# ToKe79/nuts333

Measured on AMD Instinct MI355X. Metric: delivered_broadcast_lines_per_s, higher is better.
Workload: dtype u8

## Files before the change

nuts333_amd/device/fanout.hip:

```cpp

#include <hip/hip_runtime.h>
#include <hipcub/hipcub.hpp>

#include <algorithm>
#include <chrono>
#include <cstdint>
#include <cstdio>
#include <cstring>
#include <type_traits>

namespace {

constexpr int kOutBuff = 1000;
constexpr int kTextSize = 2000;
constexpr int kNumCols = 21;
constexpr int kMaxWrites = 16;
constexpr int kBlock = 256;

constexpr uint8_t kLogin = 1, kHasRoom = 2, kSameRoom = 4, kIgnall = 8, kIgnshout = 16, kSender = 32, kColour = 64;
constexpr int kComShout = 4, kComSemote = 7;

__constant__ char kColCom[kNumCols][2] = {
    {'R', 'S'}, {'O', 'L'}, {'U', 'L'}, {'L', 'I'}, {'R', 'V'}, {'F', 'K'}, {'F', 'R'}, {'F', 'G'}, {'F', 'Y'}, {'F', 'B'},
    {'F', 'M'}, {'F', 'T'}, {'F', 'W'}, {'B', 'K'}, {'B', 'R'}, {'B', 'G'}, {'B', 'Y'}, {'B', 'B'}, {'B', 'M'}, {'B', 'T'},
    {'B', 'W'},
};
__constant__ char kColArg[kNumCols][2] = {
    {'0', 0}, {'1', 0}, {'4', 0}, {'5', 0}, {'7', 0}, {'3', '0'}, {'3', '1'}, {'3', '2'}, {'3', '3'}, {'3', '4'},
    {'3', '5'}, {'3', '6'}, {'3', '7'}, {'4', '0'}, {'4', '1'}, {'4', '2'}, {'4', '3'}, {'4', '4'}, {'4', '5'}, {'4', '6'},
    {'4', '7'},
};

__device__ __forceinline__ bool admits(uint8_t l, int rm_is_null, int force_listen, int com_num)
{
    if (l & kLogin) return false;
    if (!(l & kHasRoom)) return false;
    if (!(l & kSameRoom) && !rm_is_null) return false;
    if ((l & kIgnall) && !force_listen) return false;
    if ((l & kIgnshout) && (com_num == kComShout || com_num == kComSemote)) return false;
    if (l & kSender) return false;
    return true;
}

__device__ __forceinline__ int colcom_at(const uint8_t* s, int i, int len)
{
    if (i + 2 >= len) return -1;
    const uint8_t a = s[i + 1], b = s[i + 2];
    for (int c = 0; c < kNumCols; c++)
        if (a == (uint8_t)kColCom[c][0] && b == (uint8_t)kColCom[c][1]) return c;
    return -1;
}

template <bool EMIT>
struct Sink {
    uint8_t* out;
    int32_t* wsz;
    int64_t cap;
    int wcap;
    int64_t n = 0;
    int writes = 0;
    int pos = 0;

    __device__ __forceinline__ void put(uint8_t c)
    {
        if (EMIT && n < cap) out[n] = c;
        n++;
        pos++;
    }
    __device__ __forceinline__ void flush()
    {
        if (EMIT && writes < wcap) wsz[writes] = pos;
        writes++;
        pos = 0;
    }
    __device__ __forceinline__ void reset_code()
    {
        put(27); put('['); put('0'); put('m');
    }
};

template <bool EMIT>
__device__ void transduce(const uint8_t* s, int len, bool colour, Sink<EMIT>& k)
{
    int i = 0;
    while (i < len) {
        const uint8_t ch = s[i];
        if (ch == '\n') {
            if (k.pos > kOutBuff - 6) k.flush();
            if (colour) k.reset_code();
            k.put('\n');
            k.put('\r');
            i++;
        } else if (ch == '/' && i + 1 < len && s[i + 1] == '~') {
            i++;
            continue;
        } else if (i > 0 && ch == '~' && s[i - 1] == '/') {
            k.put('~');
            i++;
        } else if (ch == '~') {
            if (k.pos > kOutBuff - 6) k.flush();
            const int c = colcom_at(s, i, len);
            if (c >= 0) {
                if (colour) {
                    k.put(27); k.put('['); k.put((uint8_t)kColArg[c][0]);
                    if (kColArg[c][1]) k.put((uint8_t)kColArg[c][1]);
                    k.put('m');
                }
                i += 3;
            } else {
                k.put('~');
                i++;
            }
        } else {
            k.put(ch);
            i++;
        }
        if (k.pos == kOutBuff) k.flush();
    }
    if (k.pos) k.flush();
    if (colour) {
        k.reset_code();
        k.flush();
    }
}

struct Args {
    const uint8_t* text;
    const int32_t* text_off;
    const int32_t* text_len;
    const uint8_t* rec;
    int n;
    int rm_is_null, force_listen, com_num;
    uint8_t* admitted;
    int64_t* nbytes;
    int32_t* nwrites;
    int64_t* out_off;
    int32_t* w_off;
    int* violations;
    uint8_t* arena;
    int64_t arena_cap;
    int32_t* wsz;
    int64_t wsz_cap;
};

template <bool BROADCAST>
__device__ __forceinline__ bool load_item(const Args& a, int i, const uint8_t*& s, int& len)
{
    if (BROADCAST) {
        __shared__ uint8_t lds[kTextSize];
        len = a.text_len[0];
        for (int j = threadIdx.x; j < len; j += blockDim.x) lds[j] = a.text[j];
        __syncthreads();
        s = lds;
        return i < a.n;
    }
    if (i >= a.n) return false;
    s = a.text + a.text_off[i];
    len = a.text_len[i];
    return true;
}

template <bool BROADCAST>
__device__ void measure(const Args& a)
{
    const int i = blockIdx.x * blockDim.x + threadIdx.x;
    if (i == 0) {
        a.nbytes[a.n] = 0;
        a.nwrites[a.n] = 0;
    }
    const uint8_t* s;
    int len;
    if (!load_item<BROADCAST>(a, i, s, len)) return;
    const uint8_t l = a.rec[i];
    const bool in = !BROADCAST || admits(l, a.rm_is_null, a.force_listen, a.com_num);
    Sink<false> k{nullptr, nullptr, 0, 0};
    if (in) transduce(s, len, (l & kColour) != 0, k);
    if (k.n > 6 * (int64_t)len + 4 || k.writes > kMaxWrites) atomicAdd(a.violations, 1);
    a.admitted[i] = in;
    a.nbytes[i] = k.n;
    a.nwrites[i] = k.writes;
}

template <bool BROADCAST>
__device__ void emit(const Args& a)
{
    const int i = blockIdx.x * blockDim.x + threadIdx.x;
    const uint8_t* s;
    int len;
    if (!load_item<BROADCAST>(a, i, s, len) || !a.admitted[i]) return;
    const int64_t room = a.arena_cap - a.out_off[i], wroom = a.wsz_cap - a.w_off[i];
    const int64_t cap = a.nbytes[i] < room ? a.nbytes[i] : (room > 0 ? room : 0);
    const int wcap = (int)(a.nwrites[i] < wroom ? a.nwrites[i] : (wroom > 0 ? wroom : 0));
    Sink<true> k{a.arena + a.out_off[i], a.wsz + a.w_off[i], cap, wcap};
    transduce(s, len, (a.rec[i] & kColour) != 0, k);
}

constexpr int kVarCap = 6 * (kTextSize - 1) + 4;
constexpr int kGroup = 16;

struct ManyArgs {
    const uint8_t* text;
    const int32_t* text_off;
    const int32_t* text_len;
    const uint8_t* flags;
    const int32_t* com_num;
    const int32_t* item_off;
    const int32_t* tile_off;
    const uint8_t* rec;
    int k, m;
    int* violations;
    uint8_t* admitted;
    int64_t* out_off;
    int32_t* w_off;
    int64_t* nbytes;
    int32_t* nwrites;
    uint8_t* arena;
    int64_t arena_cap;
    int32_t* wsz;
    int64_t wsz_cap;
};

struct Tile {
    int b, lo, hi;
};

__device__ __forceinline__ Tile find_tile(const ManyArgs& a)
{
    const int blk = (int)blockIdx.x;
    int lo = 0, hi = a.k;
    while (hi - lo > 1) {
        const int mid = (lo + hi) >> 1;
        if (a.tile_off[mid] <= blk) lo = mid;
        else hi = mid;
    }
    const int first = a.item_off[lo] + (blk - a.tile_off[lo]) * kBlock;
    const int end = a.item_off[lo + 1];
    return {lo, first, first + kBlock < end ? first + kBlock : end};
}

template <bool EMIT, typename A>
__device__ __forceinline__ void stage_variants(const A& a, int b, uint8_t* text, uint8_t* var, int32_t* vwsz,
                                               int64_t* vn, int* vw)
{
    const int len = a.text_len[b];
    const uint8_t* src = a.text + a.text_off[b];
    for (int j = threadIdx.x; j < len; j += blockDim.x) text[j] = src[j];
    __syncthreads();
    if (threadIdx.x == 0 || threadIdx.x == 64) {
        const int c = threadIdx.x >> 6;
        Sink<EMIT> k{EMIT ? var + c * kVarCap : nullptr, EMIT ? vwsz + c * kMaxWrites : nullptr, 6 * (int64_t)len + 4,
                     kMaxWrites};
        transduce(text, len, c != 0, k);
        vn[c] = k.n;
        vw[c] = k.writes;
    }
    __syncthreads();
}

__device__ void measure_many(const ManyArgs& a)
{
    __shared__ uint8_t text[kTextSize];
    __shared__ int64_t vn[2];
    __shared__ int vw[2];
    if (blockIdx.x == 0 && threadIdx.x == 0) {
        a.nbytes[a.m] = 0;
        a.nwrites[a.m] = 0;
    }
    const Tile t = find_tile(a);
    stage_variants<false>(a, t.b, text, nullptr, nullptr, vn, vw);
    const int i = t.lo + (int)threadIdx.x;
    if (i >= t.hi) return;
    const uint8_t l = a.rec[i];
    const int fl = a.flags[t.b];
    const bool in = admits(l, fl & 1, (fl >> 1) & 1, a.com_num[t.b]);
    const int c = (l & kColour) ? 1 : 0;
    const int64_t nb = in ? vn[c] : 0;
    const int nw = in ? vw[c] : 0;
    if (nb > 6 * (int64_t)a.text_len[t.b] + 4 || nw > kMaxWrites) atomicAdd(a.violations, 1);
    a.admitted[i] = in;
    a.nbytes[i] = nb;
    a.nwrites[i] = nw;
}

__device__ void emit_many(const ManyArgs& a)
{
    __shared__ uint8_t text[kTextSize];
    __shared__ uint8_t var[2 * kVarCap];
    __shared__ int32_t vwsz[2 * kMaxWrites];
    __shared__ int64_t vn[2];
    __shared__ int vw[2];
    __shared__ int64_t s_off[kBlock], s_n[kBlock];
    __shared__ int32_t s_woff[kBlock], s_nw[kBlock];
    __shared__ uint8_t s_c[kBlock];
    const Tile t = find_tile(a);
    const int len = a.text_len[t.b];
    {
        const int i = t.lo + (int)threadIdx.x;
        if (i < t.hi) {
            const bool in = a.admitted[i] != 0;
            const int64_t off = a.out_off[i], woff = a.w_off[i];
            const int64_t room = a.arena_cap - off, wroom = a.wsz_cap - woff;
            int64_t n = in ? a.nbytes[i] : 0;
            n = n < room ? n : room;
            n = n < 6 * (int64_t)len + 4 ? n : 6 * (int64_t)len + 4;
            int64_t nw = in ? a.nwrites[i] : 0;
            nw = nw < wroom ? nw : wroom;
            nw = nw < kMaxWrites ? nw : kMaxWrites;
            s_off[threadIdx.x] = off;
            s_n[threadIdx.x] = n > 0 ? n : 0;
            s_woff[threadIdx.x] = (int32_t)woff;
            s_nw[threadIdx.x] = nw > 0 ? (int32_t)nw : 0;
            s_c[threadIdx.x] = (a.rec[i] & kColour) ? 1 : 0;
        }
    }
    stage_variants<true>(a, t.b, text, var, vwsz, vn, vw);
    const int g = (int)threadIdx.x / kGroup, lane = (int)threadIdx.x % kGroup;
    for (int j = g; j < t.hi - t.lo; j += kBlock / kGroup) {
        const int c = s_c[j];
        const int64_t n0 = s_n[j], vmax = vn[c] < kVarCap ? vn[c] : kVarCap;
        const int64_t n = n0 < vmax ? n0 : vmax;
        const uint8_t* src = var + c * kVarCap;
        uint8_t* dst = a.arena + s_off[j];
        const int head = (int)(s_off[j] & 3);
        for (int64_t w = 4 * lane - head; w < n; w += 4 * kGroup) {
            if (w >= 0 && w + 4 <= n) {
                const uint32_t v = (uint32_t)src[w] | (uint32_t)src[w + 1] << 8 | (uint32_t)src[w + 2] << 16 |
                                   (uint32_t)src[w + 3] << 24;
                *reinterpret_cast<uint32_t*>(dst + w) = v;
            } else {
                for (int q = 0; q < 4; q++)
                    if (w + q >= 0 && w + q < n) dst[w + q] = src[w + q];
            }
        }
        const int nw = s_nw[j] < vw[c] ? s_nw[j] : vw[c];
        if (lane < nw) a.wsz[s_woff[j] + lane] = vwsz[c * kMaxWrites + lane];
    }
}

static_assert(kGroup >= kMaxWrites, "emit_many writes an item's chunk sizes with one lane each");
static_assert(kBlock % kGroup == 0 && kBlock >= 128, "emit_many: whole lane groups; variants on waves 0 and 1");

struct RosterArgs {
    const int32_t* room;
    const uint8_t* slot;
    const uint8_t* text;
    const int32_t* text_off;
    const int32_t* text_len;
    const int32_t* rm;
    const int32_t* sender;
    const uint8_t* flags;
    const int32_t* com_num;
    int k, capacity, tiles;
    int* violations;
    uint8_t* admitted;
    int64_t* out_off;
    int32_t* w_off;
    uint8_t* var;
    int64_t* vn;
    int32_t* vw;
    int32_t* vwsz;
    uint8_t* arena;
    int64_t arena_cap;
    int32_t* wsz;
    int64_t wsz_cap;
};

__host__ __device__ __forceinline__ int64_t var_stride(int len) { return (6 * (int64_t)len + 4 + 3) & ~(int64_t)3; }
__device__ __forceinline__ int64_t var_at(const RosterArgs& a, int b) { return 12 * (int64_t)a.text_off[b] + 16 * (int64_t)b; }

__device__ void roster_measure(const RosterArgs& a)
{
    const int b = (int)blockIdx.x / a.tiles, tile = (int)blockIdx.x - b * a.tiles;
    const int j = tile * kBlock + (int)threadIdx.x;
    if (j < a.capacity) {
        const int room = a.room[j], rm = a.rm[b];
        const uint8_t l = (a.slot[j] & (kLogin | kIgnall | kIgnshout | kColour)) | (room >= 0 ? kHasRoom : 0) |
                          (rm >= 0 && room == rm ? kSameRoom : 0) | (j == a.sender[b] ? kSender : 0);
        a.admitted[b * a.capacity + j] = admits(l, rm < 0, (a.flags[b] >> 1) & 1, a.com_num[b]);
    }
    if (tile == 0) {
        __shared__ uint8_t text[kTextSize];
        __shared__ uint8_t var[2 * kVarCap];
        __shared__ int32_t vwsz[2 * kMaxWrites];
        __shared__ int64_t vn[2];
        __shared__ int vw[2];
        stage_variants<true>(a, b, text, var, vwsz, vn, vw);
        const int len = a.text_len[b];
        const int64_t cap = 6 * (int64_t)len + 4, stride = var_stride(len);
        uint8_t* dst = a.var + var_at(a, b);
        for (int c = 0; c < 2; c++) {
            const int64_t n = vn[c] < cap ? vn[c] : cap;
            for (int64_t q = threadIdx.x; q < n; q += kBlock) dst[c * stride + q] = var[c * kVarCap + q];
            const int nw = vw[c] < kMaxWrites ? vw[c] : kMaxWrites;
            if ((int)threadIdx.x < nw) a.vwsz[(2 * b + c) * kMaxWrites + threadIdx.x] = vwsz[c * kMaxWrites + threadIdx.x];
        }
        if (threadIdx.x < 2) {
            a.vn[2 * b + threadIdx.x] = vn[threadIdx.x];
            a.vw[2 * b + threadIdx.x] = vw[threadIdx.x];
            if (vn[threadIdx.x] > cap || vw[threadIdx.x] > kMaxWrites) atomicAdd(a.violations, 1);
        }
    }
}

template <typename T>
struct ItemCount {
    const uint8_t* admitted;
    const uint8_t* slot;
    const T* v;
    int capacity, m;
    __host__ __device__ T operator()(int i) const
    {
        if (i >= m || !admitted[i]) return 0;
        const int b = i / capacity;
        return v[2 * b + ((slot[i - b * capacity] & kColour) ? 1 : 0)];
    }
};

__device__ __forceinline__ void copy_items(int count, const uint8_t* var, const int32_t* vwsz, const int64_t* vn,
                                           const int* vw, const int64_t* s_off, const int64_t* s_n,
                                           const int32_t* s_woff, const int32_t* s_nw, const uint8_t* s_c,
                                           uint8_t* arena, int32_t* wsz)
{
    const int g = (int)threadIdx.x / kGroup, lane = (int)threadIdx.x % kGroup;
    for (int j = g; j < count; j += kBlock / kGroup) {
        const int c = s_c[j];
        const int64_t n0 = s_n[j], vmax = vn[c] < kVarCap ? vn[c] : kVarCap;
        const int64_t n = n0 < vmax ? n0 : vmax;
        const uint8_t* src = var + c * kVarCap;
        uint8_t* dst = arena + s_off[j];
        const int head = (int)(s_off[j] & 3);
        for (int64_t w = 4 * lane - head; w < n; w += 4 * kGroup) {
            if (w >= 0 && w + 4 <= n) {
                const uint32_t v = (uint32_t)src[w] | (uint32_t)src[w + 1] << 8 | (uint32_t)src[w + 2] << 16 |
                                   (uint32_t)src[w + 3] << 24;
                *reinterpret_cast<uint32_t*>(dst + w) = v;
            } else {
                for (int q = 0; q < 4; q++)
                    if (w + q >= 0 && w + q < n) dst[w + q] = src[w + q];
            }
        }
        const int nw = s_nw[j] < vw[c] ? s_nw[j] : vw[c];
        if (lane < nw) wsz[s_woff[j] + lane] = vwsz[c * kMaxWrites + lane];
    }
}

__device__ void roster_emit(const RosterArgs& a)
{
    __shared__ uint8_t var[2 * kVarCap];
    __shared__ int32_t vwsz[2 * kMaxWrites];
    __shared__ int64_t vn[2];
    __shared__ int vw[2];
    __shared__ int64_t s_off[kBlock], s_n[kBlock];
    __shared__ int32_t s_woff[kBlock], s_nw[kBlock];
    __shared__ uint8_t s_c[kBlock];
    const int b = (int)blockIdx.x / a.tiles, j0 = ((int)blockIdx.x - b * a.tiles) * kBlock;
    const int len = a.text_len[b];
    const int64_t cap = 6 * (int64_t)len + 4;
    {
        const int j = j0 + (int)threadIdx.x;
        if (j < a.capacity) {
            const int i = b * a.capacity + j;
            const bool in = a.admitted[i] != 0;
            const int64_t off = a.out_off[i], woff = a.w_off[i];
            const int64_t room = a.arena_cap - off, wroom = a.wsz_cap - woff;
            int64_t n = in ? a.out_off[i + 1] - off : 0;
            n = n < room ? n : room;
            n = n < cap ? n : cap;
            int64_t nw = in ? a.w_off[i + 1] - woff : 0;
            nw = nw < wroom ? nw : wroom;
            nw = nw < kMaxWrites ? nw : kMaxWrites;
            s_off[threadIdx.x] = off;
            s_n[threadIdx.x] = n > 0 ? n : 0;
            s_woff[threadIdx.x] = (int32_t)woff;
            s_nw[threadIdx.x] = nw > 0 ? (int32_t)nw : 0;
            s_c[threadIdx.x] = (a.slot[j] & kColour) ? 1 : 0;
        }
    }
    const uint8_t* src = a.var + var_at(a, b);
    const int64_t stride = var_stride(len);
    for (int c = 0; c < 2; c++) {
        const int64_t n = a.vn[2 * b + c] < cap ? a.vn[2 * b + c] : cap;
        for (int64_t q = threadIdx.x; q < n; q += kBlock) var[c * kVarCap + q] = src[c * stride + q];
        const int nw = a.vw[2 * b + c] < kMaxWrites ? a.vw[2 * b + c] : kMaxWrites;
        if ((int)threadIdx.x < nw) vwsz[c * kMaxWrites + threadIdx.x] = a.vwsz[(2 * b + c) * kMaxWrites + threadIdx.x];
        if (threadIdx.x == 0) {
            vn[c] = n;
            vw[c] = nw;
        }
    }
    __syncthreads();
    const int count = a.capacity - j0 < kBlock ? a.capacity - j0 : kBlock;
    copy_items(count, var, vwsz, vn, vw, s_off, s_n, s_woff, s_nw, s_c, a.arena, a.wsz);
}

static_assert(2 * kMaxWrites <= kBlock, "roster kernels move a broadcast's chunk sizes with one lane each");

struct PlanArgs {
    const int32_t* room;
    const uint8_t* slot;
    const uint8_t* text;
    const int32_t* text_off;
    const int32_t* text_len;
    const int32_t* rm;
    const int32_t* sender;
    const uint8_t* flags;
    const int32_t* com_num;
    int k, capacity, tiles;
    int words;
    int* violations;
    int64_t* vn;
    int32_t* vw;
    int32_t* vwsz;
    uint64_t* bits;
    uint8_t* var;
};

__device__ __forceinline__ int64_t var_at(const PlanArgs& a, int b) { return 12 * (int64_t)a.text_off[b] + 16 * (int64_t)b; }

__device__ void roster_plan(const PlanArgs& a)
{
    const int b = (int)blockIdx.x / a.tiles, tile = (int)blockIdx.x - b * a.tiles;
    const int j = tile * kBlock + (int)threadIdx.x;
    bool in = false;
    if (j < a.capacity) {
        const int room = a.room[j], rm = a.rm[b];
        const uint8_t l = (a.slot[j] & (kLogin | kIgnall | kIgnshout | kColour)) | (room >= 0 ? kHasRoom : 0) |
                          (rm >= 0 && room == rm ? kSameRoom : 0) | (j == a.sender[b] ? kSender : 0);
        in = admits(l, rm < 0, (a.flags[b] >> 1) & 1, a.com_num[b]);
    }
    const uint64_t word = __ballot(in);
    const int w = j >> 6;
    if ((threadIdx.x & 63) == 0 && w < a.words) a.bits[(int64_t)b * a.words + w] = word;
    if (tile == 0) {
        __shared__ uint8_t text[kTextSize];
        __shared__ uint8_t var[2 * kVarCap];
        __shared__ int32_t vwsz[2 * kMaxWrites];
        __shared__ int64_t vn[2];
        __shared__ int vw[2];
        stage_variants<true>(a, b, text, var, vwsz, vn, vw);
        const int len = a.text_len[b];
        const int64_t cap = 6 * (int64_t)len + 4, stride = var_stride(len);
        uint8_t* dst = a.var + var_at(a, b);
        for (int c = 0; c < 2; c++) {
            const int64_t n = vn[c] < cap ? vn[c] : cap;
            for (int64_t q = threadIdx.x; q < n; q += kBlock) dst[c * stride + q] = var[c * kVarCap + q];
            const int nw = vw[c] < kMaxWrites ? vw[c] : kMaxWrites;
            if ((int)threadIdx.x < nw) a.vwsz[(2 * b + c) * kMaxWrites + threadIdx.x] = vwsz[c * kMaxWrites + threadIdx.x];
        }
        if (threadIdx.x < 2) {
            a.vn[2 * b + threadIdx.x] = vn[threadIdx.x];
            a.vw[2 * b + threadIdx.x] = vw[threadIdx.x];
            if (vn[threadIdx.x] > cap || vw[threadIdx.x] > kMaxWrites) atomicAdd(a.violations, 1);
        }
    }
}

static_assert(kBlock % 64 == 0, "roster_plan: a tile is whole bitmap words, one per wave");

constexpr int kRevLines = 15;
constexpr int kRevLen = 200;
constexpr int kRevSlot = kRevLen + 2;
constexpr int kRevRing = kRevLines * kRevSlot;
constexpr int kRevLineCap = 6 * (kRevLen + 1) + 4;
constexpr int kRevLineStride = (kRevLineCap + 1 + 3) & ~3;
constexpr int kRevLineWrites = 3;
constexpr int kRevVarCap = kRevLines * kRevLineCap;
constexpr int kRevVarStride = (kRevVarCap + 3) & ~3;
constexpr int kRevWrites = kRevLines * kRevLineWrites;
constexpr int kRevTasks = 2 * kRevLines;
constexpr int kWaveLimit = kOutBuff - 6;
constexpr uint8_t kRecordBit = 4;
constexpr int kMaxReviewRooms = 1024;

struct RecordArgs {
    const uint8_t* text;
    const int32_t* text_off;
    const int32_t* text_len;
    const int32_t* rm;
    const uint8_t* flags;
    const uint8_t* clear;
    int k, review_rooms;
    uint8_t* rings;
    int32_t* revline;
};

__device__ void roster_record(const RecordArgs& a)
{
    __shared__ int s_surv[kRevLines];
    __shared__ int s_count, s_base;
    const int room = (int)blockIdx.x;
    const bool cleared = a.clear && a.clear[room];
    if (threadIdx.x < 64) {
        const int lane = (int)threadIdx.x;
        int count = 0;
        for (int b0 = 0; b0 < a.k; b0 += 64) {
            const int b = b0 + lane;
            const bool hit = b < a.k && (a.flags[b] & kRecordBit) && a.rm[b] == room;
            const uint64_t word = __ballot(hit);
            const int n = __popcll(word);
            const int rank = count + __popcll(word & ((1ull << lane) - 1));
            if (hit && rank >= count + n - kRevLines) s_surv[rank % kRevLines] = b;
            count += n;
        }
        if (lane == 0) {
            s_count = count;
            s_base = cleared ? 0 : (int)((uint32_t)a.revline[room] % kRevLines);
        }
    }
    __syncthreads();
    const int count = s_count, base = s_base;
    if (!count && !cleared) return;
    uint8_t* ring = a.rings + (size_t)room * kRevRing;
    const int nsurv = count < kRevLines ? count : kRevLines;
    const int first = (count - nsurv) % kRevLines;
    if (cleared && threadIdx.x < kRevLines) {
        const int d = ((int)threadIdx.x - base - first + 2 * kRevLines) % kRevLines;
        if (d >= nsurv) ring[threadIdx.x * kRevSlot] = 0;
    }
    for (int idx = (int)threadIdx.x; idx < nsurv * kRevSlot; idx += kBlock) {
        const int j = idx / kRevSlot, i = idx - j * kRevSlot;
        const int r = (first + j) % kRevLines;
        const int b = s_surv[r];
        uint8_t v = 0;
        if (i < kRevLen) {
            if (i < a.text_len[b]) v = a.text[a.text_off[b] + i];
        } else if (i == kRevLen) {
            v = '\n';
        }
        ring[((base + r) % kRevLines) * kRevSlot + i] = v;
    }
    if (threadIdx.x == 0) a.revline[room] = (base + count % kRevLines) % kRevLines;
}

struct ReviewArgs {
    uint8_t* rings;
    int32_t* revline;
    const int32_t* rooms;
    const uint8_t* clear;
    int q, review_rooms;
    int* violations;
    int32_t* line_count;
    int32_t* sequential;
    int32_t* vn;
    int32_t* vw;
    int32_t* vwsz;
    uint8_t* lines;
    uint8_t* var;
};

__device__ __forceinline__ int expand_byte(uint8_t p1, uint8_t ch, uint8_t n1, bool consumed, int own, bool colour,
                                           uint64_t* v)
{
    *v = ch;
    if (ch == 0 || consumed) return 0;
    if (ch == '\n') {
        if (colour) {
            *v = 27ull | (uint64_t)'[' << 8 | (uint64_t)'0' << 16 | (uint64_t)'m' << 24 | (uint64_t)'\n' << 32 |
                 (uint64_t)'\r' << 40;
            return 6;
        }
        *v = (uint64_t)'\n' | (uint64_t)'\r' << 8;
        return 2;
    }
    if (ch == '/' && n1 == '~') return 0;
    if (ch == '~' && p1 != '/' && own >= 0) {
        if (!colour) return 0;
        const uint64_t a0 = (uint8_t)kColArg[own][0], a1 = (uint8_t)kColArg[own][1];
        *v = 27ull | (uint64_t)'[' << 8 | a0 << 16 | (a1 ? a1 << 24 | (uint64_t)'m' << 32 : (uint64_t)'m' << 24);
        return a1 ? 5 : 4;
    }
    return 1;
}

__device__ void roster_review(const ReviewArgs& a)
{
    if ((int)blockIdx.x >= a.q) {
        const int room = ((int)blockIdx.x - a.q) * kBlock + (int)threadIdx.x;
        if (a.clear && room < a.review_rooms && a.clear[room]) {
            for (int i = 0; i < kRevLines; i++) a.rings[(size_t)room * kRevRing + i * kRevSlot] = 0;
            a.revline[room] = 0;
        }
        return;
    }
    __shared__ uint8_t s_line[kRevLines][kRevSlot + 2];
    __shared__ uint8_t s_out[kRevTasks][kRevLineStride];
    __shared__ int32_t s_wsz[kRevTasks][kRevLineWrites + 1];
    __shared__ int s_n[kRevTasks], s_w[kRevTasks], s_off[kRevTasks], s_woff[kRevTasks];
    __shared__ int s_len[kRevLines], s_seq;
    const int q = (int)blockIdx.x, room = a.rooms[q];
    const bool cleared = a.clear && a.clear[room];
    const int rev = cleared ? 0 : (int)((uint32_t)a.revline[room] % kRevLines);
    const uint8_t* ring = a.rings + (size_t)room * kRevRing;
    for (int idx = (int)threadIdx.x; idx < kRevRing; idx += kBlock) {
        const int i = idx / kRevSlot, j = idx - i * kRevSlot;
        const uint8_t v = cleared ? 0 : ring[((rev + i) % kRevLines) * kRevSlot + j];
        s_line[i][j] = v;
        a.lines[(size_t)q * kRevRing + idx] = v;
    }
    if (threadIdx.x == 0) s_seq = 0;
    __syncthreads();

    const int lane = (int)threadIdx.x & 63;
    for (int t = (int)threadIdx.x >> 6; t < kRevTasks; t += kBlock / 64) {
        const int i = t >> 1;
        const bool colour = (t & 1) != 0;
        const uint8_t* s = s_line[i];
        uint8_t w[9];
#pragma unroll
        for (int x = 0; x < 9; x++) {
            const int at = 4 * lane - 3 + x;
            w[x] = at >= 0 && at < kRevSlot ? s[at] : 0;
        }
        const int nul = w[3] == 0 ? 0 : w[4] == 0 ? 1 : w[5] == 0 ? 2 : w[6] == 0 ? 3 : 4;
        const uint64_t ends = __ballot(nul < 4);
        const int end_lane = __ffsll((unsigned long long)ends) - 1;
        const int len = 4 * end_lane + __shfl(nul, end_lane, 64);
#pragma unroll
        for (int x = 0; x < 9; x++)
            if (4 * lane - 3 + x >= len) w[x] = 0;
        int cmd[6], key[6];
        bool tilde = false;
#pragma unroll
        for (int x = 0; x < 6; x++) {
            cmd[x] = -1;
            key[x] = w[x + 1] == '~' && w[x] != '/' ? w[x + 2] << 8 | w[x + 3] : -1;
            tilde |= key[x] >= 0;
        }
        if (tilde) {
#pragma unroll 1
            for (int c = 0; c < kNumCols; c++) {
                const int pair = (uint8_t)kColCom[c][0] << 8 | (uint8_t)kColCom[c][1];
#pragma unroll
                for (int x = 0; x < 6; x++) cmd[x] = key[x] == pair ? c : cmd[x];
            }
        }
        int n[4], mine = 0;
        uint64_t v[4];
#pragma unroll
        for (int x = 0; x < 4; x++) {
            n[x] = expand_byte(w[x + 2], w[x + 3], w[x + 4], cmd[x] >= 0 || cmd[x + 1] >= 0, cmd[x + 2], colour, &v[x]);
            mine += n[x];
        }
        int incl = mine;
#pragma unroll
        for (int d = 1; d < 64; d <<= 1) {
            const int y = __shfl_up(incl, d, 64);
            if (lane >= d) incl += y;
        }
        const int body = __shfl(incl, 63, 64);
        uint8_t* out = s_out[t];
        if (len == 0) {
            if (lane == 0) {
                s_n[t] = 0;
                s_w[t] = 0;
            }
        } else if (body <= kWaveLimit) {
            int at = incl - mine;
#pragma unroll
            for (int x = 0; x < 4; x++) {
#pragma unroll
                for (int y = 0; y < 6; y++)
                    out[y < n[x] ? at + y : kRevLineStride - 1] = (uint8_t)(v[x] >> (8 * y));
                at += n[x];
            }
            if (colour && lane < 4) out[body + lane] = lane == 0 ? 27 : lane == 1 ? '[' : lane == 2 ? '0' : 'm';
            if (lane == 0) {
                int nw = 0;
                if (body) s_wsz[t][nw++] = body;
                if (colour) s_wsz[t][nw++] = 4;
                s_n[t] = body + (colour ? 4 : 0);
                s_w[t] = nw;
            }
        } else if (lane == 0) {
            s_n[t] = -1;
        }
        if (lane == 0 && !colour) s_len[i] = len;
    }
    __syncthreads();
    if (threadIdx.x < kRevTasks && s_n[threadIdx.x] < 0) {
        const int t = (int)threadIdx.x;
        Sink<true> k{s_out[t], s_wsz[t], kRevLineCap, kRevLineWrites};
        transduce(s_line[t >> 1], s_len[t >> 1], (t & 1) != 0, k);
        if (k.n > kRevLineCap || k.writes > kRevLineWrites) atomicAdd(a.violations, 1);
        s_n[t] = k.n < kRevLineCap ? (int)k.n : kRevLineCap;
        s_w[t] = k.writes < kRevLineWrites ? k.writes : kRevLineWrites;
        atomicAdd(&s_seq, 1);
    }
    __syncthreads();
    if (threadIdx.x < kRevTasks) {
        const int t = (int)threadIdx.x;
        int off = 0, woff = 0;
        for (int j = t & 1; j < t; j += 2) {
            off += s_n[j];
            woff += s_w[j];
        }
        s_off[t] = off;
        s_woff[t] = woff;
        if (t >= kRevTasks - 2) {
            a.vn[2 * q + (t & 1)] = off + s_n[t];
            a.vw[2 * q + (t & 1)] = woff + s_w[t];
        }
    }
    if (threadIdx.x == 64) {
        int lines = 0;
        for (int i = 0; i < kRevLines; i++) lines += s_len[i] > 0;
        a.line_count[q] = lines;
        a.sequential[q] = s_seq;
    }
    __syncthreads();
    for (int t = 0; t < kRevTasks; t++) {
        const int var = 2 * q + (t & 1);
        uint8_t* dst = a.var + (size_t)var * kRevVarStride + s_off[t];
        for (int j = (int)threadIdx.x; j < s_n[t]; j += kBlock) dst[j] = s_out[t][j];
        if ((int)threadIdx.x < s_w[t]) a.vwsz[var * kRevWrites + s_woff[t] + (int)threadIdx.x] = s_wsz[t][threadIdx.x];
    }
}

static_assert(kBlock / 64 >= 1 && 64 * 4 >= kRevSlot, "roster_review: a wave holds a whole slot, four bytes per lane");
static_assert(kBlock >= kRevTasks + 64 && kBlock >= kRevLines, "roster_review / roster_record: a lane per task, per line");

}

extern "C" __global__ void __launch_bounds__(kBlock) nuts_fanout_measure_batch(Args a) { measure<false>(a); }
extern "C" __global__ void __launch_bounds__(kBlock) nuts_fanout_measure_broadcast(Args a) { measure<true>(a); }
extern "C" __global__ void __launch_bounds__(kBlock) nuts_fanout_emit_batch(Args a) { emit<false>(a); }
extern "C" __global__ void __launch_bounds__(kBlock) nuts_fanout_emit_broadcast(Args a) { emit<true>(a); }
extern "C" __global__ void __launch_bounds__(kBlock) nuts_fanout_measure_many(ManyArgs a) { measure_many(a); }
extern "C" __global__ void __launch_bounds__(kBlock) nuts_fanout_emit_many(ManyArgs a) { emit_many(a); }
extern "C" __global__ void __launch_bounds__(kBlock) nuts_roster_measure(RosterArgs a) { roster_measure(a); }
extern "C" __global__ void __launch_bounds__(kBlock) nuts_roster_emit(RosterArgs a) { roster_emit(a); }
extern "C" __global__ void __launch_bounds__(kBlock) nuts_roster_plan(PlanArgs a) { roster_plan(a); }
extern "C" __global__ void __launch_bounds__(kBlock) nuts_roster_record(RecordArgs a) { roster_record(a); }
extern "C" __global__ void __launch_bounds__(kBlock) nuts_roster_review(ReviewArgs a) { roster_review(a); }


namespace {

struct Buffers {
    uint8_t* d_block = nullptr;
    size_t cap_block = 0, cap_host_arena = 0, cap_host_writes = 0;
    uint8_t* h_arena = nullptr;
    int32_t* h_wsz = nullptr;
    hipStream_t stream = nullptr;
    hipEvent_t ev0 = nullptr, ev1 = nullptr;
    bool ready = false;
};
Buffers g;
char g_err[512];

int fail(const char* what, hipError_t e)
{
    snprintf(g_err, sizeof(g_err), "%s: %s", what, hipGetErrorString(e));
    return -1;
}

#define ND_CHECK(call)                                  \
    do {                                                \
        hipError_t e_ = (call);                         \
        if (e_ != hipSuccess) return fail(#call, e_);   \
    } while (0)

template <typename T>
int grow_dev(T** p, size_t* cap, size_t want, const char* what)
{
    if (want <= *cap) return 0;
    if (*p) (void)hipFree(*p);
    *p = nullptr;
    *cap = 0;
    hipError_t e = hipMalloc((void**)p, want * sizeof(T));
    if (e != hipSuccess) return fail(what, e);
    *cap = want;
    return 0;
}

template <typename T>
int grow_host(T** p, size_t* cap, size_t want, const char* what)
{
    if (want <= *cap) return 0;
    if (*p) (void)hipHostFree(*p);
    *p = nullptr;
    *cap = 0;
    hipError_t e = hipHostMalloc((void**)p, want * sizeof(T), hipHostMallocDefault);
    if (e != hipSuccess) return fail(what, e);
    *cap = want;
    return 0;
}

int ensure_ready()
{
    if (g.ready) return 0;
    int n = 0;
    ND_CHECK(hipGetDeviceCount(&n));
    if (n < 1) {
        snprintf(g_err, sizeof(g_err), "no GPU visible");
        return -1;
    }
    ND_CHECK(hipSetDevice(0));
    ND_CHECK(hipStreamCreateWithFlags(&g.stream, hipStreamNonBlocking));
    ND_CHECK(hipEventCreate(&g.ev0));
    ND_CHECK(hipEventCreate(&g.ev1));
    g.ready = true;
    return 0;
}

size_t layout(uintptr_t base, size_t text_bytes, size_t scan_bytes, Args& a, uint8_t** scan)
{
    size_t at = 0;
    auto take = [&](auto*& p, size_t count) {
        p = reinterpret_cast<std::remove_reference_t<decltype(p)>>(base + at);
        at += (count * sizeof(*p) + 255) & ~(size_t)255;
    };
    const size_t n = (size_t)a.n;
    take(a.text, text_bytes);
    take(a.text_off, n);
    take(a.text_len, n);
    take(a.rec, n);
    take(a.admitted, n);
    take(a.nbytes, n + 1);
    take(a.nwrites, n + 1);
    take(a.out_off, n + 1);
    take(a.w_off, n + 1);
    take(a.violations, 1);
    take(a.arena, (size_t)a.arena_cap);
    take(a.wsz, (size_t)a.wsz_cap);
    take(*scan, scan_bytes);
    return at;
}

double now_ns()
{
    return (double)std::chrono::duration_cast<std::chrono::nanoseconds>(
               std::chrono::steady_clock::now().time_since_epoch()).count();
}

struct ManyHost {
    uint8_t* stage = nullptr;
    uint8_t* res = nullptr;
    size_t cap_stage = 0, cap_res = 0;
};
ManyHost gm;

size_t layout_many(uintptr_t base, size_t text_bytes, size_t scan_bytes, ManyArgs& a, uint8_t** scan)
{
    size_t at = 0;
    auto take = [&](auto*& p, size_t count) {
        p = reinterpret_cast<std::remove_reference_t<decltype(p)>>(base + at);
        at += (count * sizeof(*p) + 255) & ~(size_t)255;
    };
    const size_t k = (size_t)a.k, m = (size_t)a.m;
    take(a.text, text_bytes);
    take(a.text_off, k);
    take(a.text_len, k);
    take(a.flags, k);
    take(a.com_num, k);
    take(a.item_off, k + 1);
    take(a.tile_off, k + 1);
    take(a.rec, m);
    take(a.violations, 1);
    take(a.admitted, m);
    take(a.out_off, m + 1);
    take(a.w_off, m + 1);
    take(a.nbytes, m + 1);
    take(a.nwrites, m + 1);
    take(a.arena, (size_t)a.arena_cap);
    take(a.wsz, (size_t)a.wsz_cap);
    take(*scan, scan_bytes);
    return at;
}

constexpr int kMaxRosters = 64;
constexpr int kMaxCapacity = 65536;
struct Roster {
    bool live = false;
    bool resident = false;
    int capacity = 0;
    int64_t rooms = 0;
    uint8_t* d = nullptr;
    uint8_t* mirror = nullptr;
    size_t cap_d = 0, cap_mirror = 0;
    int review_rooms = 0;
    uint8_t* rings = nullptr;
};
Roster g_rosters[kMaxRosters];

size_t revline_at(const Roster& r) { return ((size_t)r.review_rooms * kRevRing + 255) & ~(size_t)255; }
size_t rings_bytes(const Roster& r) { return revline_at(r) + (size_t)r.review_rooms * sizeof(int32_t); }

size_t layout_roster(uintptr_t base, size_t text_bytes, RosterArgs& a)
{
    size_t at = 0;
    auto take = [&](auto*& p, size_t count) {
        p = reinterpret_cast<std::remove_reference_t<decltype(p)>>(base + at);
        at += (count * sizeof(*p) + 255) & ~(size_t)255;
    };
    const size_t k = (size_t)a.k, m = k * (size_t)a.capacity;
    take(a.room, (size_t)a.capacity);
    take(a.slot, (size_t)a.capacity);
    take(a.text, text_bytes);
    take(a.text_off, k);
    take(a.text_len, k);
    take(a.rm, k);
    take(a.sender, k);
    take(a.flags, k);
    take(a.com_num, k);
    take(a.violations, 1);
    take(a.admitted, m);
    take(a.out_off, m + 1);
    take(a.w_off, m + 1);
    return at;
}

size_t layout_roster_work(uintptr_t base, size_t var_bytes, size_t scan_bytes, RosterArgs& a, uint8_t** scan)
{
    size_t at = 0;
    auto take = [&](auto*& p, size_t count) {
        p = reinterpret_cast<std::remove_reference_t<decltype(p)>>(base + at);
        at += (count * sizeof(*p) + 255) & ~(size_t)255;
    };
    const size_t k = (size_t)a.k;
    take(a.var, var_bytes);
    take(a.vn, 2 * k);
    take(a.vw, 2 * k);
    take(a.vwsz, 2 * k * kMaxWrites);
    take(a.arena, (size_t)a.arena_cap);
    take(a.wsz, (size_t)a.wsz_cap);
    take(*scan, scan_bytes);
    return at;
}

size_t layout_plan(uintptr_t base, size_t text_bytes, size_t var_bytes, PlanArgs& a, size_t clear_bytes,
                   const uint8_t** clear)
{
    size_t at = 0;
    auto take = [&](auto*& p, size_t count) {
        p = reinterpret_cast<std::remove_reference_t<decltype(p)>>(base + at);
        at += (count * sizeof(*p) + 255) & ~(size_t)255;
    };
    const size_t k = (size_t)a.k;
    take(a.room, (size_t)a.capacity);
    take(a.slot, (size_t)a.capacity);
    take(a.text, text_bytes);
    take(a.text_off, k);
    take(a.text_len, k);
    take(a.rm, k);
    take(a.sender, k);
    take(a.flags, k);
    take(a.com_num, k);
    take(*clear, clear_bytes);
    take(a.violations, 1);
    take(a.vn, 2 * k);
    take(a.vw, 2 * k);
    take(a.vwsz, 2 * k * kMaxWrites);
    take(a.bits, k * (size_t)a.words);
    take(a.var, var_bytes);
    return at;
}

size_t layout_review(uintptr_t base, int capacity, size_t clear_bytes, ReviewArgs& a)
{
    size_t at = 0;
    auto take = [&](auto*& p, size_t count) {
        p = reinterpret_cast<std::remove_reference_t<decltype(p)>>(base + at);
        at += (count * sizeof(*p) + 255) & ~(size_t)255;
    };
    const size_t q = (size_t)a.q;
    const int32_t* room;
    const uint8_t* slot;
// ... 605 lines not shown
```

Measured before the change: 733,300.

## Parallelize broadcast text transduction across a wave with prefix-sum scatter

Replaces the single-thread serial transducer used to stage each broadcast's plain and colour variants with a 64-lane wave version. Each lane expands 4 bytes, looks up colour codes branch-free, and computes output offsets via a shuffle prefix sum, with the serial path kept as fallback when output exceeds one write buffer. The review path is refactored to share the same helper, and the fallback uses a branch-free colour-code lookup. This removes a long serial per-block stage at the cost of more lanes busy and extra shuffle work; outputs must match the serial write-splitting semantics.

```diff
diff --git a/nuts333_amd/device/fanout.hip b/nuts333_amd/device/fanout.hip
--- a/nuts333_amd/device/fanout.hip
+++ b/nuts333_amd/device/fanout.hip
@@ -12,6 +12,7 @@
 namespace {
 
 constexpr int kOutBuff = 1000;
+constexpr int kWaveLimit = kOutBuff - 6;
 constexpr int kTextSize = 2000;
 constexpr int kNumCols = 21;
 constexpr int kMaxWrites = 16;
@@ -42,13 +43,21 @@
     return true;
 }
 
+template <bool LADDER = true>
 __device__ __forceinline__ int colcom_at(const uint8_t* s, int i, int len)
 {
     if (i + 2 >= len) return -1;
     const uint8_t a = s[i + 1], b = s[i + 2];
+    if (LADDER) {
+        for (int c = 0; c < kNumCols; c++)
+            if (a == (uint8_t)kColCom[c][0] && b == (uint8_t)kColCom[c][1]) return c;
+        return -1;
+    }
+    int found = -1;
+#pragma unroll
     for (int c = 0; c < kNumCols; c++)
-        if (a == (uint8_t)kColCom[c][0] && b == (uint8_t)kColCom[c][1]) return c;
-    return -1;
+        found = (a << 8 | b) == ((uint8_t)kColCom[c][0] << 8 | (uint8_t)kColCom[c][1]) ? c : found;
+    return found;
 }
 
 template <bool EMIT>
@@ -79,7 +88,7 @@
     }
 };
 
-template <bool EMIT>
+template <bool EMIT, bool LADDER = true>
 __device__ void transduce(const uint8_t* s, int len, bool colour, Sink<EMIT>& k)
 {
     int i = 0;
@@ -99,7 +108,7 @@
             i++;
         } else if (ch == '~') {
             if (k.pos > kOutBuff - 6) k.flush();
-            const int c = colcom_at(s, i, len);
+            const int c = colcom_at<LADDER>(s, i, len);
             if (c >= 0) {
                 if (colour) {
                     k.put(27); k.put('['); k.put((uint8_t)kColArg[c][0]);
@@ -122,6 +131,87 @@
         k.reset_code();
         k.flush();
     }
+}
+
+__device__ __forceinline__ int expand_byte(uint8_t p1, uint8_t ch, uint8_t n1, bool consumed, int own, bool colour,
+                                           uint64_t* v)
+{
+    *v = ch;
+    if (ch == 0 || consumed) return 0;
+    if (ch == '\n') {
+        if (colour) {
+            *v = 27ull | (uint64_t)'[' << 8 | (uint64_t)'0' << 16 | (uint64_t)'m' << 24 | (uint64_t)'\n' << 32 |
+                 (uint64_t)'\r' << 40;
+            return 6;
+        }
+        *v = (uint64_t)'\n' | (uint64_t)'\r' << 8;
+        return 2;
+    }
+    if (ch == '/' && n1 == '~') return 0;
+    if (ch == '~' && p1 != '/' && own >= 0) {
+        if (!colour) return 0;
+        const uint64_t a0 = (uint8_t)kColArg[own][0], a1 = (uint8_t)kColArg[own][1];
+        *v = 27ull | (uint64_t)'[' << 8 | a0 << 16 | (a1 ? a1 << 24 | (uint64_t)'m' << 32 : (uint64_t)'m' << 24);
+        return a1 ? 5 : 4;
+    }
+    return 1;
+}
+
+template <bool EMIT>
+__device__ __forceinline__ int transduce_wave(const uint8_t* s, int len, bool colour, int lane, uint8_t* out,
+                                              uint8_t* spare)
+{
+    int body = 0;
+#pragma unroll 1
+    for (int base = 0; base < len; base += 256) {
+        uint8_t w[9];
+#pragma unroll
+        for (int x = 0; x < 9; x++) {
+            const int at = base + 4 * lane - 3 + x;
+            w[x] = at >= 0 && at < len ? s[at] : 0;
+        }
+        int cmd[6], key[6];
+        bool tilde = false;
+#pragma unroll
+        for (int x = 0; x < 6; x++) {
+            cmd[x] = -1;
+            key[x] = w[x + 1] == '~' && w[x] != '/' ? w[x + 2] << 8 | w[x + 3] : -1;
+            tilde |= key[x] >= 0;
+        }
+        if (tilde) {
+#pragma unroll 1
+            for (int c = 0; c < kNumCols; c++) {
+                const int pair = (uint8_t)kColCom[c][0] << 8 | (uint8_t)kColCom[c][1];
+#pragma unroll
+                for (int x = 0; x < 6; x++) cmd[x] = key[x] == pair ? c : cmd[x];
+            }
+        }
+        int n[4], mine = 0;
+        uint64_t v[4];
+#pragma unroll
+        for (int x = 0; x < 4; x++) {
+            n[x] = expand_byte(w[x + 2], w[x + 3], w[x + 4], cmd[x] >= 0 || cmd[x + 1] >= 0, cmd[x + 2], colour, &v[x]);
+            mine += n[x];
+        }
+        int incl = mine;
+#pragma unroll
+        for (int d = 1; d < 64; d <<= 1) {
+            const int y = __shfl_up(incl, d, 64);
+            if (lane >= d) incl += y;
+        }
+        if (EMIT) {
+            int at = body + incl - mine;
+#pragma unroll
+            for (int x = 0; x < 4; x++) {
+#pragma unroll
+                for (int y = 0; y < 6; y++)
+                    *(y < n[x] ? out + at + y : spare) = (uint8_t)(v[x] >> (8 * y));
+                at += n[x];
+            }
+        }
+        body += __shfl(incl, 63, 64);
+    }
+    return body;
 }
 
 struct Args {
@@ -246,13 +336,32 @@
     const uint8_t* src = a.text + a.text_off[b];
     for (int j = threadIdx.x; j < len; j += blockDim.x) text[j] = src[j];
     __syncthreads();
-    if (threadIdx.x == 0 || threadIdx.x == 64) {
-        const int c = threadIdx.x >> 6;
-        Sink<EMIT> k{EMIT ? var + c * kVarCap : nullptr, EMIT ? vwsz + c * kMaxWrites : nullptr, 6 * (int64_t)len + 4,
-                     kMaxWrites};
-        transduce(text, len, c != 0, k);
-        vn[c] = k.n;
-        vw[c] = k.writes;
+    if (threadIdx.x < 128) {
+        const int c = (int)threadIdx.x >> 6, lane = (int)threadIdx.x & 63;
+        uint8_t* out = EMIT ? var + c * kVarCap : nullptr;
+        int32_t* wsz = EMIT ? vwsz + c * kMaxWrites : nullptr;
+        const int body = transduce_wave<EMIT>(text, len, c != 0, lane, out, text + kTextSize - 1);
+        if (body <= kWaveLimit) {
+            if (EMIT && c && lane < 4) out[body + lane] = lane == 0 ? 27 : lane == 1 ? '[' : lane == 2 ? '0' : 'm';
+            if (lane == 0) {
+                int nw = 0;
+                if (body) {
+                    if (EMIT) wsz[nw] = body;
+                    nw++;
+                }
+                if (c) {
+                    if (EMIT) wsz[nw] = 4;
+                    nw++;
+                }
+                vn[c] = body + 4 * c;
+                vw[c] = nw;
+            }
+        } else if (lane == 0) {
+            Sink<EMIT> k{out, wsz, 6 * (int64_t)len + 4, kMaxWrites};
+            transduce<EMIT, false>(text, len, c != 0, k);
+            vn[c] = k.n;
+            vw[c] = k.writes;
+        }
     }
     __syncthreads();
 }
@@ -568,7 +677,6 @@
 constexpr int kRevVarStride = (kRevVarCap + 3) & ~3;
 constexpr int kRevWrites = kRevLines * kRevLineWrites;
 constexpr int kRevTasks = 2 * kRevLines;
-constexpr int kWaveLimit = kOutBuff - 6;
 constexpr uint8_t kRecordBit = 4;
 constexpr int kMaxReviewRooms = 1024;
 
@@ -648,30 +756,6 @@
     uint8_t* var;
 };
 
-__device__ __forceinline__ int expand_byte(uint8_t p1, uint8_t ch, uint8_t n1, bool consumed, int own, bool colour,
-                                           uint64_t* v)
-{
-    *v = ch;
-    if (ch == 0 || consumed) return 0;
-    if (ch == '\n') {
-        if (colour) {
-            *v = 27ull | (uint64_t)'[' << 8 | (uint64_t)'0' << 16 | (uint64_t)'m' << 24 | (uint64_t)'\n' << 32 |
-                 (uint64_t)'\r' << 40;
-            return 6;
-        }
-        *v = (uint64_t)'\n' | (uint64_t)'\r' << 8;
-        return 2;
-    }
-    if (ch == '/' && n1 == '~') return 0;
-    if (ch == '~' && p1 != '/' && own >= 0) {
-        if (!colour) return 0;
-        const uint64_t a0 = (uint8_t)kColArg[own][0], a1 = (uint8_t)kColArg[own][1];
-        *v = 27ull | (uint64_t)'[' << 8 | a0 << 16 | (a1 ? a1 << 24 | (uint64_t)'m' << 32 : (uint64_t)'m' << 24);
-        return a1 ? 5 : 4;
-    }
-    return 1;
-}
-
 __device__ void roster_review(const ReviewArgs& a)
 {
     if ((int)blockIdx.x >= a.q) {
@@ -705,64 +789,21 @@
         const int i = t >> 1;
         const bool colour = (t & 1) != 0;
         const uint8_t* s = s_line[i];
-        uint8_t w[9];
+        int nul = 4;
 #pragma unroll
-        for (int x = 0; x < 9; x++) {
-            const int at = 4 * lane - 3 + x;
-            w[x] = at >= 0 && at < kRevSlot ? s[at] : 0;
-        }
-        const int nul = w[3] == 0 ? 0 : w[4] == 0 ? 1 : w[5] == 0 ? 2 : w[6] == 0 ? 3 : 4;
+        for (int x = 3; x >= 0; x--)
+            if (4 * lane + x < kRevSlot && s[4 * lane + x] == 0) nul = x;
         const uint64_t ends = __ballot(nul < 4);
         const int end_lane = __ffsll((unsigned long long)ends) - 1;
         const int len = 4 * end_lane + __shfl(nul, end_lane, 64);
-#pragma unroll
-        for (int x = 0; x < 9; x++)
-            if (4 * lane - 3 + x >= len) w[x] = 0;
-        int cmd[6], key[6];
-        bool tilde = false;
-#pragma unroll
-        for (int x = 0; x < 6; x++) {
-            cmd[x] = -1;
-            key[x] = w[x + 1] == '~' && w[x] != '/' ? w[x + 2] << 8 | w[x + 3] : -1;
-            tilde |= key[x] >= 0;
-        }
-        if (tilde) {
-#pragma unroll 1
-            for (int c = 0; c < kNumCols; c++) {
-                const int pair = (uint8_t)kColCom[c][0] << 8 | (uint8_t)kColCom[c][1];
-#pragma unroll
-                for (int x = 0; x < 6; x++) cmd[x] = key[x] == pair ? c : cmd[x];
-            }
-        }
-        int n[4], mine = 0;
-        uint64_t v[4];
-#pragma unroll
-        for (int x = 0; x < 4; x++) {
-            n[x] = expand_byte(w[x + 2], w[x + 3], w[x + 4], cmd[x] >= 0 || cmd[x + 1] >= 0, cmd[x + 2], colour, &v[x]);
-            mine += n[x];
-        }
-        int incl = mine;
-#pragma unroll
-        for (int d = 1; d < 64; d <<= 1) {
-            const int y = __shfl_up(incl, d, 64);
-            if (lane >= d) incl += y;
-        }
-        const int body = __shfl(incl, 63, 64);
         uint8_t* out = s_out[t];
+        const int body = transduce_wave<true>(s, len, colour, lane, out, out + kRevLineStride - 1);
         if (len == 0) {
             if (lane == 0) {
                 s_n[t] = 0;
                 s_w[t] = 0;
             }
         } else if (body <= kWaveLimit) {
-            int at = incl - mine;
-#pragma unroll
-            for (int x = 0; x < 4; x++) {
-#pragma unroll
-                for (int y = 0; y < 6; y++)
-                    out[y < n[x] ? at + y : kRevLineStride - 1] = (uint8_t)(v[x] >> (8 * y));
-                at += n[x];
-            }
             if (colour && lane < 4) out[body + lane] = lane == 0 ? 27 : lane == 1 ? '[' : lane == 2 ? '0' : 'm';
             if (lane == 0) {
                 int nw = 0;
```

After: 728,200. No clear change (-0.7%).
